# facebookresearch/goliath

Measured on NVIDIA H100. Metric: rendered megapixels/sec (fwd+bwd) RGCA head 300k Gaussians, higher is better.
Workload: dtype f32

## Files before the change

### goliath_b200/_lib.py

```python
import ctypes
import os

import torch

_HERE = os.path.dirname(os.path.abspath(__file__))
LIB_PATH = os.path.join(_HERE, "libgoliath_b200.so")
_lib = None

_vp, _i, _f, _i64, _sz = ctypes.c_void_p, ctypes.c_int, ctypes.c_float, ctypes.c_int64, ctypes.c_size_t

SIGNATURES = {
    "gb_version": (_i, []),
    "gb_launch_count": (ctypes.c_ulonglong, []),
    "gb_launch_count_reset": (None, []),
    "gb_sg_evaluate_fwd": (_i, [_vp] * 7 + [_i] * 4 + [_vp]),
    "gb_sg_evaluate_bwd": (_i, [_vp] * 10 + [_i] * 4 + [_vp]),
    "gb_project_gaussians_fwd": (_i, [_i, _vp, _vp, _f, _vp, _vp, _f, _f, _f, _f, _i, _i, _i, _f] + [_vp] * 7 + [_vp]),
    "gb_project_gaussians_bwd": (_i, [_i, _vp, _vp, _f, _vp, _vp, _f, _f] + [_vp] * 13 + [_vp]),
    "gb_cumsum_workspace_bytes": (_sz, [_i]),
    "gb_cumsum_i32": (_i, [_i, _vp, _vp, _vp, _vp]),
    "gb_map_gaussian_to_intersects": (_i, [_i, _vp, _vp, _vp, _vp, _i, _i, _i, _vp, _vp, _vp]),
    "gb_sort_workspace_bytes": (_sz, [_i64]),
    "gb_sort_intersects": (_i, [_i64, _vp, _vp, _vp, _vp, _i, _vp, _vp]),
    "gb_get_tile_bin_edges": (_i, [_i64, _vp, _vp, _vp]),
# ... 11 lines not shown
    "gb_get_rank_sort_mode": (_i, []),
    "gb_set_rank_sort_mode": (None, [_i]),
    "gb_bin_tiles_supported": (_i, [_i]),
    "gb_bin_tiles_workspace_bytes": (_sz, [_i, _i, _i64]),
    "gb_bin_tiles_pack": (_i, [_i] + [_vp] * 7 + [_i, _i, _i, _i64] + [_vp, _vp, _i] + [_vp] * 5 + [_vp]),
    "gb_bin_tiles_pack_ev": (_i, [_i] + [_vp] * 7 + [_i, _i, _i, _i64] + [_vp, _vp, _i] + [_vp] * 5 + [_vp, _vp]),
    "gb_tile_schedule_ints": (_i, [_i]),
    "gb_tile_schedule": (_i, [_i, _vp, _vp, _vp]),
    "gb_rasterize_sched_fwd": (_i, [_i, _i, _i] + [_vp] * 7 + [_vp]),
    "gb_rasterize_sched_bwd": (_i, [_i, _i, _i] + [_vp] * 13 + [_vp]),
    "gb_records_widen": (_i, [_i64, _vp, _vp, _vp, _vp]),
    "gb_records_set_colors4": (_i, [_i64, _vp, _vp, _vp, _i, _i64, _vp, _vp]),
    "gb_rasterize_multi_fwd": (_i, [_i, _i, _vp, _vp, _i, _vp, _vp, _vp, _vp]),
    "gb_rasterize_multi_bwd": (_i, [_i, _i, _vp, _vp, _vp, _i] + [_vp] * 9 + [_vp]),
    "gb_colors12_unpack": (_i, [_i64, _i, _vp, _vp, _vp]),
    "gb_records_set_colors": (_i, [_i64] + [_vp] * 5 + [_vp]),
    "gb_splat_grad_unpack": (_i, [_i] + [_vp] * 8 + [_vp]),
    "gb_get_blend_mode": (_i, []),
    "gb_set_blend_mode": (None, [_i]),
    "gb_rasterize_packed_fwd": (_i, [_i, _i, _i] + [_vp] * 7 + [_vp]),
    "gb_rasterize_packed_bwd": (_i, [_i, _i, _i] + [_vp] * 13 + [_vp]),
    "gb_rasterize_ranked_fwd": (_i, [_i, _i, _i] + [_vp] * 8 + [_vp]),
    "gb_rasterize_ranked_bwd": (_i, [_i, _i, _i] + [_vp] * 14 + [_vp]),
    "gb_bin_tiles_ranked": (_i, [_i] + [_vp] * 7 + [_i, _i, _i, _i64] + [_vp, _vp, _i] + [_vp] * 6 + [_vp, _vp]),
    "gb_compute_raydirs_fwd": (_i, [_i, _i, _i] + [_vp] * 5 + [_f] + [_vp] * 3 + [_vp]),
    "gb_compute_raydirs_bwd": (_i, []),
    "gb_mvp_aabb_workspace_bytes": (_sz, [_i, _i]),
    "gb_mvp_compute_aabb": (_i, [_i, _i] + [_vp] * 8 + [_vp]),
    "gb_get_raymarch_mode": (_i, []),
    "gb_set_raymarch_mode": (None, [_i]),
    "gb_mvp_raymarch_fwd": (_i, [_i] * 4 + [_vp, _vp, _f] + [_vp] * 5 + [_i] * 3 + [_vp] + [_i] * 3 + [_vp] * 4
                            + [_i, _f, _f, _i, _i, _vp]),
    "gb_deconv_tc_weight_bytes": (_sz, [_i, _i]),
    "gb_nchw_to_nhwc_split": (_i, [_i] * 5 + [_vp] * 3 + [_vp]),
    "gb_deconv4x4s2_tc_fwd": (_i, [_i] * 6 + [_vp] * 6 + [_f, _i, _vp, _vp, _i, _vp, _vp]),
    "gb_deconv4x4s2_wnub_fwd": (_i, [_i] * 5 + [_vp] * 4 + [_f, _i, _vp, _vp]),
    "gb_deconv4x4s2_wnub_bwd": (_i, [_i] * 5 + [_vp] * 5 + [_f, _i] + [_vp] * 4 + [_vp]),
    "gb_conv4x4s2_wnub_fwd": (_i, [_i] * 5 + [_vp] * 4 + [_f, _i, _vp, _vp]),
    "gb_conv4x4s2_wnub_bwd": (_i, [_i] * 5 + [_vp] * 5 + [_f, _i] + [_vp] * 4 + [_vp]),
    "gb_conv2d_wnub_fwd": (_i, [_i] * 6 + [_vp] * 4 + [_i, _f, _i, _vp, _vp]),
    "gb_conv2d_wnub_bwd": (_i, [_i] * 6 + [_vp] * 5 + [_f, _i, _i] + [_vp] * 4 + [_vp]),
    "gb_mvp_slab_to_prims_fwd": (_i, [_i] * 6 + [_vp] * 3 + [_f, _f, _i, _vp, _vp]),
    "gb_mvp_slab_to_prims_bwd": (_i, [_i] * 6 + [_vp] * 3 + [_f, _f, _i] + [_vp] * 3 + [_vp]),
    "gb_mvp_prim_transform_fwd": (_i, [_i, _i] + [_vp] * 3 + [_f, _i] + [_vp] * 3 + [_vp]),
    "gb_mvp_prim_transform_bwd": (_i, [_i, _i] + [_vp] * 3 + [_f, _i] + [_vp] * 4 + [_vp]),
    "gb_mvp_prim_frames_fwd": (_i, [_i] * 4 + [_vp] * 10 + [_vp]),
# ... 76 lines not shown
```

### goliath_b200/csrc/splat_blend_mom.cu

```cuda
#include <cstdlib>
#include <cstring>

#include "common.cuh"
#include "splat_blend_common.cuh"

namespace {

using namespace gbblend;

constexpr int kPixelWarps = 8;
constexpr int kStageRecs = 128;
constexpr int kFwdStages = 4;
constexpr int kFwdThreads = (kPixelWarps + 1) * 32;
constexpr int kBwdStages = 3;
constexpr int kBwdThreads = kPixelWarps * 32;
constexpr int kChunk = 16;
constexpr int kEntryCap = 48;
constexpr int kMStride = 33;
constexpr float kCullMargin = 2e-3f;

__device__ __forceinline__ float rcp_approx(float x) {
  float r;
  asm("rcp.approx.ftz.f32 %0, %1;" : "=f"(r) : "f"(x));
  return r;
// ... 21 lines not shown
  if (q0.z > 1e30f) return true;
  const float4 q1 = *q1p;
  const float dxlo = q0.x - fx1, dxhi = q0.x - fx0, dylo = q0.y - fy1, dyhi = q0.y - fy0;
  const float ex0 = fminf(fmaxf(0.f, dxlo), dxhi), ey0 = fminf(fmaxf(0.f, dylo), dyhi);
  const float dy1 = fminf(fmaxf(-q1.y * ex0 * rcp_approx(q1.z), dylo), dyhi);
  const float dx2 = fminf(fmaxf(-q1.y * ey0 * rcp_approx(q1.x), dxlo), dxhi);
  const float f1 = 0.5f * (q1.x * ex0 * ex0 + q1.z * dy1 * dy1) + q1.y * ex0 * dy1;
  const float f2 = 0.5f * (q1.x * dx2 * dx2 + q1.z * ey0 * ey0) + q1.y * dx2 * ey0;
  const float s = __logf(255.f * q1.w);
  return fminf(f1, f2) <= s + kCullMargin + 1e-4f * fabsf(s);
}

struct Tile {
  int tile_id, tx, ty;
};
__device__ __forceinline__ Tile make_tile(int tile_id, int tbx) {
  Tile t;
  t.tile_id = tile_id;
  t.ty = tile_id / tbx;
  t.tx = tile_id - t.ty * tbx;
  return t;
}

template <int C, bool LIST, bool RANKED>
__global__ void __launch_bounds__(kFwdThreads) blend_fwd_ilp_kernel(
    int img_w, int img_h, int tbx, const int* order, int sched, const int2* __restrict__ tile_bins,
    const float4* __restrict__ rec , const int* __restrict__ ranks ,
    const float* __restrict__ background, float* __restrict__ final_Ts, int* __restrict__ final_idx,
    float* __restrict__ out_img) {
  __shared__ __align__(128) float4 s_rec[kFwdStages][kStageRecs * 3];
  __shared__ __align__(8) unsigned long long s_full[kFwdStages];
  __shared__ __align__(8) unsigned long long s_empty[kFwdStages];
  __shared__ int s_ndone;
  __shared__ int s_tile;
  __shared__ __align__(16) int s_hits[LIST ? kPixelWarps : 1][LIST ? kStageRecs + 4 : 4];

  const int tr = threadIdx.x, lane = tr & 31, warp = tr >> 5;
  if (tr == 0) {
    s_tile = draw_tile(order, sched, tbx * ((img_h + 15) >> 4));
#pragma unroll
    for (int s = 0; s < kFwdStages; ++s) {
      mbar_init(&s_full[s], RANKED ? 32 : 1);
      mbar_init(&s_empty[s], kPixelWarps);
    }
    s_ndone = 0;
    fence_mbar_init();
  }
  __syncthreads();
  if (s_tile < 0) return;
  const Tile tl = make_tile(s_tile, tbx);
  const int2 range = tile_bins[tl.tile_id];
  const int num_batches = (range.y - range.x + kStageRecs - 1) / kStageRecs;
// ... 49 lines not shown
        if (*ndone >= kPixelWarps) break;
      }
      const int start = range.x + b * kStageRecs;
      const unsigned bytes = (unsigned)min(kStageRecs, range.y - start) * kRecBytes;
      mbar_expect_tx(&s_full[s], bytes);
      bulk_g2s(&s_rec[s][0], rec + (size_t)start * 3, bytes, &s_full[s]);
      issued = b + 1;
    }
    for (int b = max(0, issued - kFwdStages); b < issued; ++b)
      mbar_wait(&s_full[b % kFwdStages], (unsigned)((b / kFwdStages) & 1));
    return;
  }

  const int wx0 = tl.tx * 16 + ((warp & 1) << 3), wy0 = tl.ty * 16 + ((warp >> 1) << 2);
  const int pxi = wx0 + (lane & 7), pyi = wy0 + (lane >> 3);
  const bool inside = (pxi < img_w) && (pyi < img_h);
  const float px = (float)pxi + 0.5f, py = (float)pyi + 0.5f;
  const float fx0 = (float)wx0 + 0.5f, fx1 = (float)wx0 + 7.5f, fy0 = (float)wy0 + 0.5f, fy1 = (float)wy0 + 3.5f;

  bool done = !inside;
  float T = 1.f;
  int cur_idx = 0;
  float acc[4] = {0.f, 0.f, 0.f, 0.f};

  bool counted = false;
  for (int b = 0; b < num_batches; ++b) {
    const bool all_done = __all_sync(0xffffffffu, done);
    if (all_done && !counted) {
      counted = true;
      if (lane == 0) atomicAdd(&s_ndone, 1);
    }
    const int s = b % kFwdStages;
    const unsigned par = (unsigned)((b / kFwdStages) & 1);
    int st = 0;
    if (lane == 0) {
      volatile int* ndone = &s_ndone;
      for (;;) {
        if (mbar_try(&s_full[s], par)) { st = 1; break; }
        if (all_done && *ndone >= kPixelWarps) { st = 2; break; }
      }
    }
    st = __shfl_sync(0xffffffffu, st, 0);
    if (st == 2) break;
    if (all_done) {
      if (lane == 0) mbar_arrive(&s_empty[s]);
      continue;
    }
    mbar_wait(&s_full[s], par);
    const float4* sr = s_rec[s];
    const int batch_start = range.x + b * kStageRecs;
    const int batch_size = min(kStageRecs, range.y - batch_start);
    if (LIST) {
      int* hl = s_hits[LIST ? warp : 0];
      const unsigned lt = (1u << lane) - 1u;
      int cnt = 0;
#pragma unroll 4
      for (int c0 = 0; c0 < batch_size; c0 += 32) {
        const int ti = c0 + lane;
        bool hit = false;
        if (ti < batch_size) hit = footprint_hit(sr[ti * 3], &sr[ti * 3 + 1], fx0, fx1, fy0, fy1);
        const unsigned mask = __ballot_sync(0xffffffffu, hit);
        if (hit) hl[cnt + __popc(mask & lt)] = ti;
        cnt += __popc(mask);
      }
      __syncwarp();
      for (int i0 = 0; i0 < cnt; i0 += 16) {
        const int i1 = min(i0 + 16, cnt);
        for (int i = i0; i < i1; i += 4) {
          const int4 e = *reinterpret_cast<const int4*>(hl + i);
          bool live[4];
          int t[4];
          live[0] = true; live[1] = i + 1 < cnt; live[2] = i + 2 < cnt; live[3] = i + 3 < cnt;
          t[0] = e.x; t[1] = live[1] ? e.y : e.x; t[2] = live[2] ? e.z : e.x; t[3] = live[3] ? e.w : e.x;
          float alpha[4], sig[4];
          float4 col[4];
#pragma unroll
          for (int u = 0; u < 4; ++u) {
            const float4 q0 = sr[t[u] * 3], q1 = sr[t[u] * 3 + 1];
            col[u] = sr[t[u] * 3 + 2];
            const float dx = q0.x - px, dy = q0.y - py;
            sig[u] = 0.5f * (q1.x * dx * dx + q1.z * dy * dy) + q1.y * dx * dy;
            alpha[u] = fminf(kAlphaMaxFwd, q1.w * exp_neg(sig[u]));
          }
#pragma unroll
          for (int u = 0; u < 4; ++u) {
            const bool ok = live[u] && !done && !(sig[u] < 0.f) && !(alpha[u] < kAlphaMin);
            const float next_T = T * (1.f - alpha[u]);
            const bool stop = ok && (next_T <= kTEps);
            const bool take = ok && !stop;
            done = done || stop;
            if (take) {
              const float vis = alpha[u] * T;
              acc[0] += col[u].x * vis;
              acc[1] += col[u].y * vis;
              acc[2] += col[u].z * vis;
              if (C == 4) acc[3] += col[u].w * vis;
              T = next_T;
              cur_idx = batch_start + t[u];
            }
          }
        }
        if (__all_sync(0xffffffffu, done)) break;
      }
    } else {
    for (int c0 = 0; c0 < batch_size; c0 += 32) {
        const int ti = c0 + lane;
        bool hit = false;
        if (ti < batch_size) hit = footprint_hit(sr[ti * 3], &sr[ti * 3 + 1], fx0, fx1, fy0, fy1);
        unsigned mask = __ballot_sync(0xffffffffu, hit);
        while (mask) {
          int t[4];
          bool live[4];
  #pragma unroll
          for (int u = 0; u < 4; ++u) {
            live[u] = mask != 0;
            t[u] = live[u] ? c0 + __ffs(mask) - 1 : t[0];
            mask &= mask - 1;
          }
          float alpha[4], sig[4];
          float4 col[4];
  #pragma unroll
          for (int u = 0; u < 4; ++u) {
            const float4 q0 = sr[t[u] * 3], q1 = sr[t[u] * 3 + 1];
            col[u] = sr[t[u] * 3 + 2];
            const float dx = q0.x - px, dy = q0.y - py;
            sig[u] = 0.5f * (q1.x * dx * dx + q1.z * dy * dy) + q1.y * dx * dy;
// ... 3 lines not shown
          for (int u = 0; u < 4; ++u) {
            const bool ok = live[u] && !done && !(sig[u] < 0.f) && !(alpha[u] < kAlphaMin);
            const float next_T = T * (1.f - alpha[u]);
            const bool stop = ok && (next_T <= kTEps);
            const bool take = ok && !stop;
            done = done || stop;
            if (take) {
              const float vis = alpha[u] * T;
              acc[0] += col[u].x * vis;
              acc[1] += col[u].y * vis;
              acc[2] += col[u].z * vis;
              if (C == 4) acc[3] += col[u].w * vis;
              T = next_T;
              cur_idx = batch_start + t[u];
            }
          }
        }
        if (__all_sync(0xffffffffu, done)) break;
      }
  }
    __syncwarp();
    if (lane == 0) mbar_arrive(&s_empty[s]);
  }
  if (inside) {
    const size_t pix = (size_t)pyi * img_w + pxi;
    final_Ts[pix] = T;
    final_idx[pix] = cur_idx;
    if (C == 4) {
      reinterpret_cast<float4*>(out_img)[pix] =
          make_float4(acc[0] + T * background[0], acc[1] + T * background[1], acc[2] + T * background[2],
                      acc[3] + T * background[3]);
    } else {
      out_img[pix * 3 + 0] = acc[0] + T * background[0];
      out_img[pix * 3 + 1] = acc[1] + T * background[1];
      out_img[pix * 3 + 2] = acc[2] + T * background[2];
    }
  }
}

constexpr int kSmRec = kBwdStages * kStageRecs * kRecBytes;
constexpr int kSmEntries = kPixelWarps * kEntryCap * 48;
constexpr int kSmM = kPixelWarps * kChunk * kMStride * 8;
constexpr int kSmVo = kPixelWarps * 32 * 16;
constexpr int kBwdSmem = kSmRec + kSmEntries + kSmM + kSmVo;

template <int C, bool RANKED>
// ... 272 lines not shown
    __syncwarp();
    int refill = 0;
    if (lane == 0) {
      __threadfence_block();
      const int ticket = atomicAdd(&s_ticket[s], 1);
      if (ticket == kPixelWarps - 1) {
        __threadfence_block();
        s_ticket[s] = 0;
        if (k + kBwdStages < num_batches) {
          if (RANKED) refill = 1;
          else issue(k + kBwdStages);
        }
      }
    }
    if (RANKED) {
      refill = __shfl_sync(0xffffffffu, refill, 0);
      if (refill) issue_ranked(k + kBwdStages);
    }
  }
  if (cnt > 0) chunk(0, pad4(cnt));
  if (RANKED) cp_async_wait_all();
}

constexpr int kMK = 4;
constexpr int kMC = 3 * kMK;
constexpr int kMRQ = 5;
constexpr int kMRecBytes = kMRQ * 16;

__global__ void __launch_bounds__(kFwdThreads) blend_fwd_multi_kernel(
    int img_w, int img_h, int tbx, const int* order, int sched, const int2* __restrict__ tile_bins,
    const float4* __restrict__ rec, const float* __restrict__ background, float* __restrict__ out_planes ) {
  __shared__ __align__(128) float4 s_rec[kFwdStages][kStageRecs * kMRQ];
  __shared__ __align__(8) unsigned long long s_full[kFwdStages];
  __shared__ __align__(8) unsigned long long s_empty[kFwdStages];
  __shared__ int s_ndone;
  __shared__ __align__(16) int s_hits[kPixelWarps][kStageRecs + 4];
  __shared__ int s_tile;

  const int tr = threadIdx.x, lane = tr & 31, warp = tr >> 5;
  if (tr == 0) {
    s_tile = draw_tile(order, sched, tbx * ((img_h + 15) >> 4));
#pragma unroll
    for (int s = 0; s < kFwdStages; ++s) {
      mbar_init(&s_full[s], 1);
      mbar_init(&s_empty[s], kPixelWarps);
    }
// ... 423 lines not shown
    if (k < nk) {
      float* dst = v_colors + ((size_t)k * G + g) * 3;
      dst[0] = v[3 * k]; dst[1] = v[3 * k + 1]; dst[2] = v[3 * k + 2];
    }
  const float4 z = make_float4(0.f, 0.f, 0.f, 0.f);
  v12[3 * g] = z; v12[3 * g + 1] = z; v12[3 * g + 2] = z;
}

bool g_multi_attr_set[64] = {};

bool g_attr_set[64] = {};

}

namespace gbblend {

static bool fwd_list_variant() {
  const char* e = getenv("GOLIATH_B200_BLEND_FWD");
  return !(e && !strcmp(e, "rounds"));
}

static int launch_fwd_any(int img_h, int img_w, int channels, const int32_t* tile_bins, const int32_t* tile_order, int sched,
                          const float* records, const int32_t* ranks, const float* background, float* out_img,
                          float* final_Ts, int32_t* final_idx, cudaStream_t s) {
  const int tbx = gb::cdiv(img_w, 16), tby = gb::cdiv(img_h, 16);
  if (sched && !tile_order) return (int)cudaErrorInvalidValue;
  static const bool list = fwd_list_variant();
#define GB_FWD_MOM(CC, LL, RR)                                                                                          \
  blend_fwd_ilp_kernel<CC, LL, RR><<<tbx * tby, kFwdThreads, 0, s>>>(img_w, img_h, tbx, tile_order, sched,              \
                                                                     (const int2*)tile_bins, (const float4*)records,    \
                                                                     ranks, background, final_Ts, final_idx, out_img)
  if (ranks) {
    if (channels == 3) GB_FWD_MOM(3, true, true); else GB_FWD_MOM(4, true, true);
  } else if (channels == 3) {
    if (list) GB_FWD_MOM(3, true, false); else GB_FWD_MOM(3, false, false);
  } else {
    if (list) GB_FWD_MOM(4, true, false); else GB_FWD_MOM(4, false, false);
  }
#undef GB_FWD_MOM
  gb::count_launches(1);
  GB_CHECK_LAUNCH();
  return 0;
}

static int launch_bwd_any(int img_h, int img_w, int channels, const int32_t* gids_sorted, const int32_t* ranks,
                          const int32_t* tile_bins, const int32_t* tile_order, int sched, const float* records,
                          const float* background, const float* final_Ts, const int32_t* final_idx, const float* v_output,
                          const float* v_output_alpha, float* v_xy, float* v_conic, float* v_colors, float* v_opacity,
                          cudaStream_t s) {
  const int tbx = gb::cdiv(img_w, 16), tby = gb::cdiv(img_h, 16);
  if (sched && !tile_order) return (int)cudaErrorInvalidValue;
  int dev = 0;
  GB_CUDA(cudaGetDevice(&dev));
  if (dev < 0 || dev >= 64 || !g_attr_set[dev]) {
    GB_CUDA(cudaFuncSetAttribute(blend_bwd_mom_kernel<3, false>, cudaFuncAttributeMaxDynamicSharedMemorySize, kBwdSmem));
    GB_CUDA(cudaFuncSetAttribute(blend_bwd_mom_kernel<4, false>, cudaFuncAttributeMaxDynamicSharedMemorySize, kBwdSmem));
    GB_CUDA(cudaFuncSetAttribute(blend_bwd_mom_kernel<3, true>, cudaFuncAttributeMaxDynamicSharedMemorySize, kBwdSmem));
    GB_CUDA(cudaFuncSetAttribute(blend_bwd_mom_kernel<4, true>, cudaFuncAttributeMaxDynamicSharedMemorySize, kBwdSmem));
    if (dev >= 0 && dev < 64) g_attr_set[dev] = true;
  }
#define GB_BWD_MOM(CC, RR)                                                                                              \
  blend_bwd_mom_kernel<CC, RR><<<tbx * tby, kBwdThreads, kBwdSmem, s>>>(                                                \
      img_w, img_h, tbx, tile_order, sched, gids_sorted, ranks, (const int2*)tile_bins, (const float4*)records, background, \
      final_Ts, final_idx, v_output, v_output_alpha, v_xy, v_conic, v_colors, v_opacity)
  if (ranks) {
    if (channels == 3) GB_BWD_MOM(3, true); else GB_BWD_MOM(4, true);
  } else {
    if (channels == 3) GB_BWD_MOM(3, false); else GB_BWD_MOM(4, false);
  }
#undef GB_BWD_MOM
  gb::count_launches(1);
  GB_CHECK_LAUNCH();
  return 0;
}

int launch_fwd_mom(int img_h, int img_w, int channels, const int32_t* tile_bins, const int32_t* tile_order, int sched,
                   const float* records, const float* background, float* out_img, float* final_Ts, int32_t* final_idx,
                   cudaStream_t s) {
  return launch_fwd_any(img_h, img_w, channels, tile_bins, tile_order, sched, records, nullptr, background, out_img, final_Ts,
                        final_idx, s);
}

int launch_bwd_mom(int img_h, int img_w, int channels, const int32_t* gids_sorted, const int32_t* tile_bins,
                   const int32_t* tile_order, int sched, const float* records, const float* background, const float* final_Ts,
                   const int32_t* final_idx, const float* v_output, const float* v_output_alpha, float* v_xy,
                   float* v_conic, float* v_colors, float* v_opacity, cudaStream_t s) {
  return launch_bwd_any(img_h, img_w, channels, gids_sorted, nullptr, tile_bins, tile_order, sched, records, background,
                        final_Ts, final_idx, v_output, v_output_alpha, v_xy, v_conic, v_colors, v_opacity, s);
}

}

GB_API int gb_rasterize_ranked_fwd(int img_h, int img_w, int channels, const int32_t* tile_bins, const int32_t* tile_order,
                                   const int32_t* ranks_sorted, const float* rec_by_rank, const float* background,
                                   float* out_img, float* final_Ts, int32_t* final_idx, void* stream) {
  if (img_h <= 0 || img_w <= 0) return 0;
  if ((channels != 3 && channels != 4) || !ranks_sorted) return (int)cudaErrorInvalidValue;
  return gbblend::launch_fwd_any(img_h, img_w, channels, tile_bins, tile_order, 0, rec_by_rank, ranks_sorted, background,
                                 out_img, final_Ts, final_idx, (cudaStream_t)stream);
}
GB_API int gb_rasterize_ranked_bwd(int img_h, int img_w, int channels, const int32_t* rank_to_gid,
                                   const int32_t* ranks_sorted, const int32_t* tile_bins, const int32_t* tile_order,
                                   const float* rec_by_rank, const float* background, const float* final_Ts,
                                   const int32_t* final_idx, const float* v_output, const float* v_output_alpha,
                                   float* v_xy, float* v_conic, float* v_colors, float* v_opacity, void* stream) {
  if (img_h <= 0 || img_w <= 0) return 0;
  if ((channels != 3 && channels != 4) || !ranks_sorted) return (int)cudaErrorInvalidValue;
  return gbblend::launch_bwd_any(img_h, img_w, channels, rank_to_gid, ranks_sorted, tile_bins, tile_order, 0, rec_by_rank,
                                 background, final_Ts, final_idx, v_output, v_output_alpha, v_xy, v_conic, v_colors,
                                 v_opacity, (cudaStream_t)stream);
}

GB_API int gb_records_widen(int64_t cap, const int32_t* n_dev, const float* records, float* records_wide, void* stream) {
  if (cap <= 0) return 0;
  records_widen_kernel<<<(unsigned)gb::cdiv64(cap, 256), 256, 0, (cudaStream_t)stream>>>(cap, n_dev, (const float4*)records,
                                                                                         (float4*)records_wide);
  gb::count_launches(1);
  GB_CHECK_LAUNCH();
  return 0;
}
GB_API int gb_records_set_colors4(int64_t cap, const int32_t* n_dev, const int32_t* gids_sorted, const float* colors, int nk,
                                  int64_t G, float* records_wide, void* stream) {
  if (cap <= 0) return 0;
  if (nk < 1 || nk > 4) return (int)cudaErrorInvalidValue;
  records_set_colors4_kernel<<<(unsigned)gb::cdiv64(cap, 256), 256, 0, (cudaStream_t)stream>>>(cap, n_dev, gids_sorted, colors, nk,
                                                                                               G, (float4*)records_wide);
  gb::count_launches(1);
  GB_CHECK_LAUNCH();
  return 0;
}
GB_API int gb_rasterize_multi_fwd(int img_h, int img_w, const int32_t* tile_bins, const int32_t* tile_order, int sched,
                                  const float* records_wide, const float* background, float* out_planes, void* stream) {
  if (img_h <= 0 || img_w <= 0) return 0;
// ... 37 lines not shown
```

### goliath_b200/gsplat/fused.py

```python
import os
from typing import NamedTuple

import torch
from torch.autograd import Function

from .. import _lib
from .project import _project_bwd, _project_fwd
from .utils import _tile_bounds, _workspace, bin_and_sort_gaussians, compute_cumulative_intersects, key_bits

_OVERFLOW = {}

BINNING = os.environ.get("GOLIATH_B200_BINNING", "buckets")
SPLIT = os.environ.get("GOLIATH_B200_RENDER_SPLIT", "1") != "0"
RANKED = os.environ.get("GOLIATH_B200_RECORDS", "ranked") == "ranked"


def _overflow_flag(dev):
    f = _OVERFLOW.get(dev.index)
    if f is None:
        f = torch.zeros(1, dtype=torch.int32, device=dev)
        _OVERFLOW[dev.index] = f
    return f


# ... 205 lines not shown
        out4 = torch.empty(H, W, 4, **f32)
        final_Ts = torch.empty(H, W, **f32)
        final_idx = torch.empty(H, W, **i32)
        bg4 = torch.cat([background, background[:1]])
        tb = _tile_bounds(H, W, 16)
        cap = int(capacity)
        plan = _blend_plan(tb[0] * tb[1])
        ev = None
        if colors_event is not None:
            ev = colors_event.cuda_event
            colors.record_stream(torch.cuda.current_stream(dev))
        if plan.ranked:
            gids = torch.empty(G, **i32)
            ranks = torch.empty(cap, **i32)
            records = torch.empty(G, 12, **f32)
            outs = (ranks, records, gids)
        else:
            gids = torch.empty(cap, **i32)
            ranks = gids
            records = torch.empty(cap, 12, **f32)
            outs = (gids, records)
        bins, order = _bin_tiles(xys, depths, radii, conics, colors, opacity, comp, H, W, cap, plan, outs,
                                 ranked=plan.ranked, colors_ready=ev)
        with torch.cuda.device(dev):
            st = _lib.stream_ptr(dev)
            if plan.ranked:
                _lib.check(L.gb_rasterize_ranked_fwd(H, W, 4, _lib.ptr(bins), _lib.ptr(order), _lib.ptr(ranks),
                                                     _lib.ptr(records), _lib.ptr(bg4), _lib.ptr(out4), _lib.ptr(final_Ts),
                                                     _lib.ptr(final_idx), st), "rasterize_ranked_forward")
            else:
                _lib.check(plan.fwd(H, W, 4, _lib.ptr(bins), _lib.ptr(order), _lib.ptr(records), _lib.ptr(bg4),
                                    _lib.ptr(out4), _lib.ptr(final_Ts), _lib.ptr(final_idx), st),
                           "rasterize_packed_forward")
        ctx.save_for_backward(opacity, comp, bg4, gids, bins, order, records, final_Ts, final_idx, ranks)
        ctx.meta = (H, W, plan)
        ctx.set_materialize_grads(False)
        return out4, 1 - final_Ts

    @staticmethod
    def backward(ctx, v_out4, v_alpha):
        opacity, comp, bg4, gids, bins, order, records, final_Ts, final_idx, ranks = ctx.saved_tensors
        H, W, plan = ctx.meta

        def blend(st, *grads):
            if plan.ranked:
                _lib.check(_lib.lib().gb_rasterize_ranked_bwd(
                    H, W, 4, _lib.ptr(gids), _lib.ptr(ranks), _lib.ptr(bins), _lib.ptr(order), _lib.ptr(records),
                    _lib.ptr(bg4), _lib.ptr(final_Ts), _lib.ptr(final_idx), *map(_lib.ptr, grads), st),
                    "rasterize_ranked_backward")
            else:
                _lib.check(plan.bwd(H, W, 4, _lib.ptr(gids), _lib.ptr(bins), _lib.ptr(order), _lib.ptr(records),
                                    _lib.ptr(bg4), _lib.ptr(final_Ts), _lib.ptr(final_idx), *map(_lib.ptr, grads), st),
                           "rasterize_packed_backward")

        v_xy, v_conic, v_colors, v_opacity, v_comp, v_depth = _blend_grads(H, W, v_out4, v_alpha, opacity, comp, blend)
        return (v_xy, v_depth, v_conic, v_comp, None, v_opacity, v_colors) + (None,) * 5


def render_fused_split(means3d, scales, glob_scale, quats, viewmat, fx, fy, cx, cy, img_height, img_width, opacity, colors,
                       background, clip_thresh, capacity, colors_event=None):
    xys, depths, conics, comp, radii = _ProjectGeom.apply(means3d, scales, quats, viewmat, glob_scale, fx, fy, cx, cy,
                                                          img_height, img_width, clip_thresh)
    out4, alpha = _BinBlend.apply(xys, depths, conics, comp, radii, opacity, colors, background, img_height, img_width,
                                  capacity, colors_event)
    return out4, alpha, radii


def render_fused(means3d, scales, glob_scale, quats, viewmat, fx, fy, cx, cy, img_height, img_width, opacity, colors,
                 background, clip_thresh=0.01, capacity=None, colors_event=None):
    if (capacity is not None and SPLIT and BINNING == "buckets" and means3d.size(0) > 0
            and _lib.lib().gb_bin_tiles_supported(means3d.size(0))):
        return render_fused_split(means3d, scales, glob_scale, quats, viewmat, fx, fy, cx, cy, img_height, img_width,
# ... 6 lines not shown
```

### include/goliath_b200.h

```cpp
#ifndef GOLIATH_B200_H_
#define GOLIATH_B200_H_

#include <stddef.h>
#include <stdint.h>

#ifdef __cplusplus
extern "C" {
#endif

int gb_version(void);
unsigned long long gb_launch_count(void);
void gb_launch_count_reset(void);


int gb_sg_evaluate_fwd(const float* lobe_dirs, const float* lobe_sigmas, const float* light_values,
                       const float* light_pts, const float* prim_pts, const int32_t* n_lights, float* integral,
                       int N, int D, int L, int w_type, void* stream);

int gb_sg_evaluate_bwd(const float* lobe_dirs, const float* lobe_sigmas, const float* light_values,
                       const float* light_pts, const float* prim_pts, const int32_t* n_lights,
                       const float* grad_integral, float* grad_dirs, float* grad_sigmas, float* grad_light_values,
                       int N, int D, int L, int w_type, void* stream);


// ... 82 lines not shown
                      const float* colors3, const float* opacity, const float* compensation, int img_h, int img_w,
                      int block_width, int64_t cap, int32_t* tile_bins, int32_t* tile_order, int tile_sched,
                      int32_t* gids_sorted, float* records, int32_t* n_out, int32_t* overflow, void* workspace,
                      void* stream);
int gb_bin_tiles_pack_ev(int G, const float* xys, const float* depths, const int32_t* radii, const float* conics,
                         const float* colors3, const float* opacity, const float* compensation, int img_h, int img_w,
                         int block_width, int64_t cap, int32_t* tile_bins, int32_t* tile_order, int tile_sched,
                         int32_t* gids_sorted, float* records, int32_t* n_out, int32_t* overflow, void* workspace,
                         void* colors_ready, void* stream);

int gb_bin_tiles_ranked(int G, const float* xys, const float* depths, const int32_t* radii, const float* conics,
                        const float* colors3, const float* opacity, const float* compensation, int img_h, int img_w,
                        int block_width, int64_t cap, int32_t* tile_bins, int32_t* tile_order, int tile_sched,
                        int32_t* ranks_sorted, float* rec_by_rank, int32_t* rank_to_gid, int32_t* n_out, int32_t* overflow,
                        void* workspace, void* colors_ready, void* stream);
int gb_rasterize_ranked_fwd(int img_h, int img_w, int channels, const int32_t* tile_bins, const int32_t* tile_order,
                            const int32_t* ranks_sorted, const float* rec_by_rank, const float* background,
                            float* out_img, float* final_Ts, int32_t* final_idx, void* stream);
int gb_rasterize_ranked_bwd(int img_h, int img_w, int channels, const int32_t* rank_to_gid, const int32_t* ranks_sorted,
                            const int32_t* tile_bins, const int32_t* tile_order, const float* rec_by_rank,
                            const float* background, const float* final_Ts, const int32_t* final_idx,
                            const float* v_output, const float* v_output_alpha, float* v_xy, float* v_conic,
                            float* v_colors, float* v_opacity, void* stream);

int gb_tile_order(int num_tiles, const int32_t* tile_bins, int32_t* order, void* stream);

int gb_get_blend_mode(void);
void gb_set_blend_mode(int mode);

int gb_tile_schedule_ints(int num_tiles);
int gb_tile_schedule(int num_tiles, const int32_t* tile_bins, int32_t* sched, void* stream);
int gb_rasterize_sched_fwd(int img_h, int img_w, int channels, const int32_t* tile_bins, int32_t* sched,
                           const float* records, const float* background, float* out_img, float* final_Ts,
                           int32_t* final_idx, void* stream);
int gb_rasterize_sched_bwd(int img_h, int img_w, int channels, const int32_t* gids_sorted, const int32_t* tile_bins,
                           int32_t* sched, const float* records, const float* background, const float* final_Ts,
                           const int32_t* final_idx, const float* v_output, const float* v_output_alpha, float* v_xy,
                           float* v_conic, float* v_colors, float* v_opacity, void* stream);

int gb_rasterize_packed_fwd(int img_h, int img_w, int channels, const int32_t* tile_bins, const int32_t* tile_order,
                            const float* records, const float* background, float* out_img, float* final_Ts,
                            int32_t* final_idx, void* stream);

int gb_rasterize_packed_bwd(int img_h, int img_w, int channels, const int32_t* gids_sorted,
                            const int32_t* tile_bins, const int32_t* tile_order, const float* records,
                            const float* background, const float* final_Ts, const int32_t* final_idx,
// ... 179 lines not shown
```

Measured before the change: 1518.

## Record per-warp hit lists in forward and replay them in backward blend

The forward blend kernel now writes each warp's list of Gaussians that actually passed the coverage test, plus a per-warp count, into new buffers. A new backward kernel walks only those recorded hits in reverse instead of re-scanning every Gaussian in the tile. It also takes work items dynamically from a queue ordered by list length, so long lists start first. This adds forward-pass writes and an 8x-capacity hit buffer in memory, and needs an extra single-block ordering kernel launch.

New measurement: 1596, median of 6. 1.05x the previous value.

```diff
diff --git a/goliath_b200/_lib.py b/goliath_b200/_lib.py
--- a/goliath_b200/_lib.py
+++ b/goliath_b200/_lib.py
@@ -57,6 +57,8 @@
     "gb_rasterize_packed_bwd": (_i, [_i, _i, _i] + [_vp] * 13 + [_vp]),
     "gb_rasterize_ranked_fwd": (_i, [_i, _i, _i] + [_vp] * 8 + [_vp]),
     "gb_rasterize_ranked_bwd": (_i, [_i, _i, _i] + [_vp] * 14 + [_vp]),
+    "gb_rasterize_ranked_fwd_lists": (_i, [_i, _i, _i] + [_vp] * 10 + [_vp]),
+    "gb_rasterize_ranked_bwd_lists": (_i, [_i, _i, _i] + [_vp] * 14 + [_vp]),
     "gb_bin_tiles_ranked": (_i, [_i] + [_vp] * 7 + [_i, _i, _i, _i64] + [_vp, _vp, _i] + [_vp] * 6 + [_vp, _vp]),
     "gb_compute_raydirs_fwd": (_i, [_i, _i, _i] + [_vp] * 5 + [_f] + [_vp] * 3 + [_vp]),
     "gb_compute_raydirs_bwd": (_i, []),
diff --git a/goliath_b200/csrc/splat_blend_mom.cu b/goliath_b200/csrc/splat_blend_mom.cu
--- a/goliath_b200/csrc/splat_blend_mom.cu
+++ b/goliath_b200/csrc/splat_blend_mom.cu
@@ -67,12 +67,13 @@
   return t;
 }
 
-template <int C, bool LIST, bool RANKED>
+template <int C, bool LIST, bool RANKED, bool HITS = false>
 __global__ void __launch_bounds__(kFwdThreads) blend_fwd_ilp_kernel(
     int img_w, int img_h, int tbx, const int* order, int sched, const int2* __restrict__ tile_bins,
     const float4* __restrict__ rec , const int* __restrict__ ranks ,
     const float* __restrict__ background, float* __restrict__ final_Ts, int* __restrict__ final_idx,
-    float* __restrict__ out_img) {
+    float* __restrict__ out_img, int* __restrict__ hit_list = nullptr, int* __restrict__ hit_count = nullptr) {
+  static_assert(!HITS || LIST, "hit lists are the LIST variant's per-stage lists");
   __shared__ __align__(128) float4 s_rec[kFwdStages][kStageRecs * 3];
   __shared__ __align__(8) unsigned long long s_full[kFwdStages];
   __shared__ __align__(8) unsigned long long s_empty[kFwdStages];
@@ -168,6 +169,8 @@
   float T = 1.f;
   int cur_idx = 0;
   float acc[4] = {0.f, 0.f, 0.f, 0.f};
+  int* const seg = HITS ? hit_list + 8 * (size_t)range.x + (size_t)warp * (range.y - range.x) : nullptr;
+  int written = 0, last_pos = -1;
 
   bool counted = false;
   for (int b = 0; b < num_batches; ++b) {
@@ -210,6 +213,10 @@
         cnt += __popc(mask);
       }
       __syncwarp();
+      if (HITS) {
+        for (int i = lane; i < cnt; i += 32) seg[written + i] = batch_start + hl[i];
+        if (b == 0 && range.x == 0 && cnt > 0 && hl[0] == 0 && inside) last_pos = 0;
+      }
       for (int i0 = 0; i0 < cnt; i0 += 16) {
         const int i1 = min(i0 + 16, cnt);
         for (int i = i0; i < i1; i += 4) {
@@ -243,11 +250,13 @@
               if (C == 4) acc[3] += col[u].w * vis;
               T = next_T;
               cur_idx = batch_start + t[u];
+              if (HITS) last_pos = written + i + u;
             }
           }
         }
         if (__all_sync(0xffffffffu, done)) break;
       }
+      written += cnt;
     } else {
     for (int c0 = 0; c0 < batch_size; c0 += 32) {
         const int ti = c0 + lane;
@@ -297,6 +306,12 @@
     __syncwarp();
     if (lane == 0) mbar_arrive(&s_empty[s]);
   }
+  if (HITS) {
+#pragma unroll
+    for (int o = 16; o > 0; o >>= 1) last_pos = max(last_pos, __shfl_xor_sync(0xffffffffu, last_pos, o));
+    if (lane == 0) hit_count[8 * tl.tile_id + warp] = last_pos + 1;
+    if (blockIdx.x == 0 && tr == 0) hit_count[8 * tbx * ((img_h + 15) >> 4)] = 0;
+  }
   if (inside) {
     const size_t pix = (size_t)pyi * img_w + pxi;
     final_Ts[pix] = T;
@@ -615,6 +630,237 @@
   if (RANKED) cp_async_wait_all();
 }
 
+constexpr int kListWarps = 4;
+constexpr int kListThreads = kListWarps * 32;
+constexpr int kOrderBuckets = 64;
+
+__device__ __forceinline__ void cp_async_commit() { asm volatile("cp.async.commit_group;" ::: "memory"); }
+
+__global__ void __launch_bounds__(1024) order_items_kernel(int n_items, int* __restrict__ hit_count) {
+  __shared__ int s_off[kOrderBuckets];
+  const int tr = threadIdx.x, lane = tr & 31;
+  auto bucket = [](int n) { return kOrderBuckets - 1 - min((n + kChunk - 1) / kChunk, kOrderBuckets - 1); };
+  if (tr < kOrderBuckets) s_off[tr] = 0;
+  __syncthreads();
+  for (int i = tr; i < n_items; i += blockDim.x) {
+    const int n = hit_count[i];
+    if (n > 0) atomicAdd(&s_off[bucket(n)], 1);
+  }
+  __syncthreads();
+  if (tr < 32) {
+    const int a = s_off[2 * lane], b = s_off[2 * lane + 1];
+    int incl = a + b;
+#pragma unroll
+    for (int o = 1; o < 32; o <<= 1) {
+      const int t = __shfl_up_sync(0xffffffffu, incl, o);
+      if (lane >= o) incl += t;
+    }
+    const int excl = incl - a - b;
+    s_off[2 * lane] = excl;
+    s_off[2 * lane + 1] = excl + a;
+    if (lane == 31) hit_count[n_items + 1] = incl;
+  }
+  __syncthreads();
+  int* items = hit_count + n_items + 2;
+  for (int i = tr; i < n_items; i += blockDim.x) {
+    const int n = hit_count[i];
+    if (n > 0) items[atomicAdd(&s_off[bucket(n)], 1)] = i;
+  }
+}
+
+template <int C>
+__global__ void __launch_bounds__(kListThreads, 6) blend_bwd_lists_kernel(
+    int img_w, int img_h, int tbx, int n_items, const int2* __restrict__ tile_bins, const int* __restrict__ hit_list,
+    const int* __restrict__ hit_count, int* draw ,
+    const int* __restrict__ ranks, const float4* __restrict__ rec, const float* __restrict__ background,
+    const float* __restrict__ final_Ts, const int* __restrict__ final_idx, const float* __restrict__ v_output,
+    const float* __restrict__ v_output_alpha, float* __restrict__ v_xy, float* __restrict__ v_conic,
+    float* __restrict__ v_colors, float* __restrict__ v_opacity) {
+  __shared__ __align__(16) float4 s_e[kListWarps][2][kChunk * 3];
+  __shared__ __align__(8) int2 s_ig[kListWarps][2][kChunk];
+  __shared__ float2 s_m[kListWarps][kChunk * kMStride];
+  __shared__ float4 s_vo[kListWarps][32];
+
+  const int lane = threadIdx.x & 31, wib = threadIdx.x >> 5;
+  float2* M = s_m[wib];
+  float4* VO = s_vo[wib];
+  const int n_work = hit_count[n_items + 1];
+  const int* items = hit_count + n_items + 2;
+  const int n_draws = n_work + (int)gridDim.x * kListWarps;
+  for (;;) {
+    int k = 0;
+    if (lane == 0) {
+      k = atomicAdd(draw, 1);
+      if (k == n_draws - 1) *draw = 0;
+    }
+    k = __shfl_sync(0xffffffffu, k, 0);
+    if (k >= n_work) break;
+    const int item = items[k], tile = item >> 3, warp = item & 7;
+    const int n = hit_count[item];
+    const int2 range = tile_bins[tile];
+    const int* list = hit_list + 8 * (size_t)range.x + (size_t)warp * (range.y - range.x);
+    const Tile tl = make_tile(tile, tbx);
+    const int wx0 = tl.tx * 16 + ((warp & 1) << 3), wy0 = tl.ty * 16 + ((warp >> 1) << 2);
+    const int pxi = wx0 + (lane & 7), pyi = wy0 + (lane >> 3);
+    const bool inside = (pxi < img_w) && (pyi < img_h);
+    const float px = (float)pxi + 0.5f, py = (float)pyi + 0.5f;
+    const float fx0 = (float)wx0 + 0.5f, fy0 = (float)wy0 + 0.5f;
+    const size_t pix = inside ? ((size_t)pyi * img_w + pxi) : 0;
+
+    const int nchunks = (n + kChunk - 1) / kChunk;
+    int g_idx = 0, g_id = 0;
+    auto load_next = [&](int j) {
+      const int top = n - kChunk * j;
+      if (lane < min(kChunk, top)) {
+        g_idx = list[top - 1 - lane];
+        g_id = ranks[g_idx];
+      }
+    };
+    auto gather = [&](int j) {
+      const int cnt = min(kChunk, n - kChunk * j);
+      float4* E = s_e[wib][j & 1];
+      if (lane < cnt) {
+        const float4* src = rec + 3 * (size_t)g_id;
+        cp_async16(&E[lane * 3 + 0], src);
+        cp_async16(&E[lane * 3 + 1], src + 1);
+        cp_async16(&E[lane * 3 + 2], src + 2);
+        s_ig[wib][j & 1][lane] = make_int2(g_idx, g_id);
+      } else if (lane < ((cnt + 3) & ~3)) {
+        E[lane * 3 + 0] = make_float4(0.f, 0.f, 0.f, 0.f);
+        E[lane * 3 + 1] = make_float4(1.f, 0.f, 1.f, 0.f);
+        E[lane * 3 + 2] = make_float4(0.f, 0.f, 0.f, 0.f);
+        s_ig[wib][j & 1][lane] = make_int2(0x7fffffff, 0);
+      }
+      cp_async_commit();
+    };
+    load_next(0);
+    gather(0);
+
+    const float T_final = inside ? final_Ts[pix] : 1.f;
+    float T = T_final;
+    float bufv = 0.f;
+    const int bin_final = inside ? final_idx[pix] : -1;
+    float vo[4] = {0.f, 0.f, 0.f, 0.f};
+    float voa = 0.f;
+    if (inside) {
+#pragma unroll
+      for (int c = 0; c < C; ++c) vo[c] = v_output[pix * C + c];
+      voa = v_output_alpha ? v_output_alpha[pix] : 0.f;
+    }
+    VO[lane] = make_float4(vo[0], vo[1], vo[2], vo[3]);
+    float bgdot = 0.f;
+#pragma unroll
+    for (int c = 0; c < C; ++c) bgdot += background[c] * vo[c];
+    const float tfc = T_final * (voa - bgdot);
+    if (nchunks > 1) load_next(1);
+
+    for (int j = 0; j < nchunks; ++j) {
+      const int cnt = min(kChunk, n - kChunk * j);
+      const int nn = j + 1 < nchunks ? kChunk : ((cnt + 3) & ~3);
+      const float4* E = s_e[wib][j & 1];
+      const int2* IG = s_ig[wib][j & 1];
+      cp_async_wait_all();
+      __syncwarp();
+#pragma unroll 1
+      for (int h0 = 0; h0 < nn; h0 += 4) {
+        float al[4], ov[4], ra[4];
+        float4 col[4];
+#pragma unroll
+        for (int u = 0; u < 4; ++u) {
+          const int h = h0 + u;
+          const float4 q0 = E[h * 3], q1 = E[h * 3 + 1];
+          col[u] = E[h * 3 + 2];
+          const float dx = q0.x - px, dy = q0.y - py;
+          const float sigma = 0.5f * (q1.x * dx * dx + q1.z * dy * dy) + q1.y * dx * dy;
+          const float vis = exp_neg(sigma);
+          const float alpha = fminf(kAlphaMaxBwd, q1.w * vis);
+          const bool valid = (IG[h].x <= bin_final) && !(sigma < 0.f) && !(alpha < kAlphaMin);
+          al[u] = valid ? alpha : 0.f;
+          ov[u] = valid ? q1.w * vis : 0.f;
+          ra[u] = rcp_approx(1.f - al[u]);
+        }
+#pragma unroll
+        for (int u = 0; u < 4; ++u) {
+          const float cc[4] = {col[u].x, col[u].y, col[u].z, col[u].w};
+          float cv = 0.f;
+#pragma unroll
+          for (int c = 0; c < C; ++c) cv += cc[c] * vo[c];
+          const float v_alpha = ((cv * T - bufv) + tfc) * ra[u];
+          T *= ra[u];
+          const float fac = al[u] * T;
+          bufv += cv * fac;
+          M[(h0 + u) * kMStride + lane] = make_float2(fac, -ov[u] * v_alpha);
+        }
+      }
+      if (j + 1 < nchunks) {
+        gather(j + 1);
+        if (j + 2 < nchunks) load_next(j + 2);
+      }
+      __syncwarp();
+      {
+        const int hh = lane & 15, half = lane >> 4;
+        const int he = min(hh, nn - 1);
+        const float4 q0 = E[he * 3], q1 = E[he * 3 + 1];
+        const int e_id = IG[he].y;
+        const float2* Mrow = M + hh * kMStride + half * 16;
+        const float4* V = VO + half * 16;
+        float g[4] = {0.f, 0.f, 0.f, 0.f};
+        float r00 = 0.f, r01 = 0.f, r10 = 0.f, r11 = 0.f, sii = 0.f;
+        float facmax = 0.f;
+#pragma unroll
+        for (int q = 0; q < 16; ++q) {
+          const float2 m = Mrow[q];
+          const float4 v = V[q];
+          const float fi = (float)(q & 7);
+          facmax = fmaxf(facmax, m.x);
+          g[0] += m.x * v.x;
+          g[1] += m.x * v.y;
+          g[2] += m.x * v.z;
+          if (C == 4) g[3] += m.x * v.w;
+          if (q < 8) {
+            r00 += m.y;
+            r10 += m.y * fi;
+          } else {
+            r01 += m.y;
+            r11 += m.y * fi;
+          }
+          sii += m.y * (fi * fi);
+        }
+        const float u_ = q0.x - fx0, v_ = q0.y - (fy0 + (float)(2 * half));
+        const float S0 = r00 + r01, Sj = r01, Si = r10 + r11, Sij = r11;
+        const float sx = u_ * S0 - Si, sy = v_ * S0 - Sj;
+        const float sxx = u_ * (u_ * S0 - 2.f * Si) + sii;
+        const float sxy = u_ * (v_ * S0 - Sj) - v_ * Si + Sij;
+        const float syy = v_ * (v_ * S0 - 2.f * Sj) + Sj;
+        float o[10];
+        o[0] = g[0]; o[1] = g[1]; o[2] = g[2]; o[3] = g[3];
+        o[4] = 0.5f * sxx; o[5] = sxy; o[6] = 0.5f * syy;
+        o[7] = q1.x * sx + q1.y * sy;
+        o[8] = q1.y * sx + q1.z * sy;
+        o[9] = S0;
+#pragma unroll
+        for (int i = 0; i < 10; ++i) o[i] += __shfl_xor_sync(0xffffffffu, o[i], 16);
+        facmax = fmaxf(facmax, __shfl_xor_sync(0xffffffffu, facmax, 16));
+        if (half == 0 && hh < nn && facmax > 0.f) {
+          if (C == 4) {
+            gb::red_add_v4(v_colors + 4 * (size_t)e_id, o[0], o[1], o[2], o[3]);
+          } else {
+            gb::red_add(v_colors + 3 * (size_t)e_id + 0, o[0]);
+            gb::red_add(v_colors + 3 * (size_t)e_id + 1, o[1]);
+            gb::red_add(v_colors + 3 * (size_t)e_id + 2, o[2]);
+          }
+          gb::red_add(v_conic + 3 * (size_t)e_id + 0, o[4]);
+          gb::red_add(v_conic + 3 * (size_t)e_id + 1, o[5]);
+          gb::red_add(v_conic + 3 * (size_t)e_id + 2, o[6]);
+          gb::red_add_v2(v_xy + 2 * (size_t)e_id, o[7], o[8]);
+          gb::red_add(v_opacity + e_id, -o[9] * rcp_approx(q1.w));
+        }
+      }
+      __syncwarp();
+    }
+  }
+}
+
 constexpr int kMK = 4;
 constexpr int kMC = 3 * kMK;
 constexpr int kMRQ = 5;
@@ -1084,15 +1330,18 @@
 
 static int launch_fwd_any(int img_h, int img_w, int channels, const int32_t* tile_bins, const int32_t* tile_order, int sched,
                           const float* records, const int32_t* ranks, const float* background, float* out_img,
-                          float* final_Ts, int32_t* final_idx, cudaStream_t s) {
+                          float* final_Ts, int32_t* final_idx, cudaStream_t s, int32_t* hit_list = nullptr,
+                          int32_t* hit_count = nullptr) {
   const int tbx = gb::cdiv(img_w, 16), tby = gb::cdiv(img_h, 16);
   if (sched && !tile_order) return (int)cudaErrorInvalidValue;
   static const bool list = fwd_list_variant();
-#define GB_FWD_MOM(CC, LL, RR)                                                                                          \
-  blend_fwd_ilp_kernel<CC, LL, RR><<<tbx * tby, kFwdThreads, 0, s>>>(img_w, img_h, tbx, tile_order, sched,              \
-                                                                     (const int2*)tile_bins, (const float4*)records,    \
-                                                                     ranks, background, final_Ts, final_idx, out_img)
-  if (ranks) {
+#define GB_FWD_MOM(CC, LL, RR, ...)                                                                                     \
+  blend_fwd_ilp_kernel<CC, LL, RR, ##__VA_ARGS__><<<tbx * tby, kFwdThreads, 0, s>>>(                                   \
+      img_w, img_h, tbx, tile_order, sched, (const int2*)tile_bins, (const float4*)records, ranks, background, final_Ts, \
+      final_idx, out_img, hit_list, hit_count)
+  if (ranks && hit_list) {
+    if (channels == 3) GB_FWD_MOM(3, true, true, true); else GB_FWD_MOM(4, true, true, true);
+  } else if (ranks) {
     if (channels == 3) GB_FWD_MOM(3, true, true); else GB_FWD_MOM(4, true, true);
   } else if (channels == 3) {
     if (list) GB_FWD_MOM(3, true, false); else GB_FWD_MOM(3, false, false);
@@ -1136,6 +1385,41 @@
   return 0;
 }
 
+static int launch_bwd_lists(int img_h, int img_w, int channels, const int32_t* ranks, const int32_t* tile_bins,
+                            const int32_t* hit_list, int32_t* hit_count, const float* records,
+                            const float* background, const float* final_Ts, const int32_t* final_idx,
+                            const float* v_output, const float* v_output_alpha, float* v_xy, float* v_conic,
+                            float* v_colors, float* v_opacity, cudaStream_t s) {
+  const int tbx = gb::cdiv(img_w, 16), tby = gb::cdiv(img_h, 16);
+  const int n_items = 8 * tbx * tby;
+  int dev = 0;
+  GB_CUDA(cudaGetDevice(&dev));
+  static int resident[64][2] = {};
+  int uncached = 0;
+  int& per_sm = (dev >= 0 && dev < 64) ? resident[dev][channels == 4] : uncached;
+  if (per_sm == 0) {
+    int n = 0, sms = 0;
+    if (channels == 4)
+      GB_CUDA(cudaOccupancyMaxActiveBlocksPerMultiprocessor(&n, blend_bwd_lists_kernel<4>, kListThreads, 0));
+    else
+      GB_CUDA(cudaOccupancyMaxActiveBlocksPerMultiprocessor(&n, blend_bwd_lists_kernel<3>, kListThreads, 0));
+    GB_CUDA(cudaDeviceGetAttribute(&sms, cudaDevAttrMultiProcessorCount, dev));
+    per_sm = max(1, n) * sms;
+  }
+  const int grid = min(per_sm, gb::cdiv(n_items, kListWarps));
+  order_items_kernel<<<1, 1024, 0, s>>>(n_items, hit_count);
+#define GB_BWD_LISTS(CC)                                                                                                \
+  blend_bwd_lists_kernel<CC><<<grid, kListThreads, 0, s>>>(                                                             \
+      img_w, img_h, tbx, n_items, (const int2*)tile_bins, hit_list, hit_count, hit_count + n_items, ranks,              \
+      (const float4*)records, background, final_Ts, final_idx, v_output, v_output_alpha, v_xy, v_conic, v_colors,       \
+      v_opacity)
+  if (channels == 3) GB_BWD_LISTS(3); else GB_BWD_LISTS(4);
+#undef GB_BWD_LISTS
+  gb::count_launches(2);
+  GB_CHECK_LAUNCH();
+  return 0;
+}
+
 int launch_fwd_mom(int img_h, int img_w, int channels, const int32_t* tile_bins, const int32_t* tile_order, int sched,
                    const float* records, const float* background, float* out_img, float* final_Ts, int32_t* final_idx,
                    cudaStream_t s) {
@@ -1171,6 +1455,26 @@
   return gbblend::launch_bwd_any(img_h, img_w, channels, rank_to_gid, ranks_sorted, tile_bins, tile_order, 0, rec_by_rank,
                                  background, final_Ts, final_idx, v_output, v_output_alpha, v_xy, v_conic, v_colors,
                                  v_opacity, (cudaStream_t)stream);
+}
+GB_API int gb_rasterize_ranked_fwd_lists(int img_h, int img_w, int channels, const int32_t* tile_bins,
+                                         const int32_t* tile_order, const int32_t* ranks_sorted, const float* rec_by_rank,
+                                         const float* background, float* out_img, float* final_Ts, int32_t* final_idx,
+                                         int32_t* hit_list, int32_t* hit_count, void* stream) {
+  if (img_h <= 0 || img_w <= 0) return 0;
+  if ((channels != 3 && channels != 4) || !ranks_sorted || !hit_list || !hit_count) return (int)cudaErrorInvalidValue;
+  return gbblend::launch_fwd_any(img_h, img_w, channels, tile_bins, tile_order, 0, rec_by_rank, ranks_sorted, background,
+                                 out_img, final_Ts, final_idx, (cudaStream_t)stream, hit_list, hit_count);
+}
+GB_API int gb_rasterize_ranked_bwd_lists(int img_h, int img_w, int channels, const int32_t* ranks_sorted,
+                                         const int32_t* tile_bins, const int32_t* hit_list, int32_t* hit_count,
+                                         const float* rec_by_rank, const float* background, const float* final_Ts,
+                                         const int32_t* final_idx, const float* v_output, const float* v_output_alpha,
+                                         float* v_xy, float* v_conic, float* v_colors, float* v_opacity, void* stream) {
+  if (img_h <= 0 || img_w <= 0) return 0;
+  if ((channels != 3 && channels != 4) || !ranks_sorted || !hit_list || !hit_count) return (int)cudaErrorInvalidValue;
+  return gbblend::launch_bwd_lists(img_h, img_w, channels, ranks_sorted, tile_bins, hit_list, hit_count,
+                                   rec_by_rank, background, final_Ts, final_idx, v_output, v_output_alpha, v_xy, v_conic,
+                                   v_colors, v_opacity, (cudaStream_t)stream);
 }
 
 GB_API int gb_records_widen(int64_t cap, const int32_t* n_dev, const float* records, float* records_wide, void* stream) {
diff --git a/goliath_b200/gsplat/fused.py b/goliath_b200/gsplat/fused.py
--- a/goliath_b200/gsplat/fused.py
+++ b/goliath_b200/gsplat/fused.py
@@ -251,32 +251,38 @@
             outs = (gids, records)
         bins, order = _bin_tiles(xys, depths, radii, conics, colors, opacity, comp, H, W, cap, plan, outs,
                                  ranked=plan.ranked, colors_ready=ev)
+        hit_list = hit_count = None
         with torch.cuda.device(dev):
             st = _lib.stream_ptr(dev)
             if plan.ranked:
-                _lib.check(L.gb_rasterize_ranked_fwd(H, W, 4, _lib.ptr(bins), _lib.ptr(order), _lib.ptr(ranks),
-                                                     _lib.ptr(records), _lib.ptr(bg4), _lib.ptr(out4), _lib.ptr(final_Ts),
-                                                     _lib.ptr(final_idx), st), "rasterize_ranked_forward")
+                hit_list = torch.empty(8 * cap, **i32)
+                hit_count = torch.empty(16 * tb[0] * tb[1] + 2, **i32)
+                _lib.check(L.gb_rasterize_ranked_fwd_lists(H, W, 4, _lib.ptr(bins), _lib.ptr(order), _lib.ptr(ranks),
+                                                           _lib.ptr(records), _lib.ptr(bg4), _lib.ptr(out4),
+                                                           _lib.ptr(final_Ts), _lib.ptr(final_idx), _lib.ptr(hit_list),
+                                                           _lib.ptr(hit_count), st), "rasterize_ranked_forward")
             else:
                 _lib.check(plan.fwd(H, W, 4, _lib.ptr(bins), _lib.ptr(order), _lib.ptr(records), _lib.ptr(bg4),
                                     _lib.ptr(out4), _lib.ptr(final_Ts), _lib.ptr(final_idx), st),
                            "rasterize_packed_forward")
-        ctx.save_for_backward(opacity, comp, bg4, gids, bins, order, records, final_Ts, final_idx, ranks)
+        ctx.save_for_backward(opacity, comp, bg4, gids, bins, order, records, final_Ts, final_idx, ranks, hit_list,
+                              hit_count)
         ctx.meta = (H, W, plan)
         ctx.set_materialize_grads(False)
         return out4, 1 - final_Ts
 
     @staticmethod
     def backward(ctx, v_out4, v_alpha):
-        opacity, comp, bg4, gids, bins, order, records, final_Ts, final_idx, ranks = ctx.saved_tensors
+        (opacity, comp, bg4, gids, bins, order, records, final_Ts, final_idx, ranks, hit_list,
+         hit_count) = ctx.saved_tensors
         H, W, plan = ctx.meta
 
         def blend(st, *grads):
             if plan.ranked:
-                _lib.check(_lib.lib().gb_rasterize_ranked_bwd(
-                    H, W, 4, _lib.ptr(gids), _lib.ptr(ranks), _lib.ptr(bins), _lib.ptr(order), _lib.ptr(records),
-                    _lib.ptr(bg4), _lib.ptr(final_Ts), _lib.ptr(final_idx), *map(_lib.ptr, grads), st),
-                    "rasterize_ranked_backward")
+                _lib.check(_lib.lib().gb_rasterize_ranked_bwd_lists(
+                    H, W, 4, _lib.ptr(ranks), _lib.ptr(bins), _lib.ptr(hit_list),
+                    _lib.ptr(hit_count), _lib.ptr(records), _lib.ptr(bg4), _lib.ptr(final_Ts), _lib.ptr(final_idx),
+                    *map(_lib.ptr, grads), st), "rasterize_ranked_backward")
             else:
                 _lib.check(plan.bwd(H, W, 4, _lib.ptr(gids), _lib.ptr(bins), _lib.ptr(order), _lib.ptr(records),
                                     _lib.ptr(bg4), _lib.ptr(final_Ts), _lib.ptr(final_idx), *map(_lib.ptr, grads), st),
diff --git a/include/goliath_b200.h b/include/goliath_b200.h
--- a/include/goliath_b200.h
+++ b/include/goliath_b200.h
@@ -128,6 +128,16 @@
                             const float* background, const float* final_Ts, const int32_t* final_idx,
                             const float* v_output, const float* v_output_alpha, float* v_xy, float* v_conic,
                             float* v_colors, float* v_opacity, void* stream);
+int gb_rasterize_ranked_fwd_lists(int img_h, int img_w, int channels, const int32_t* tile_bins, const int32_t* tile_order,
+                                  const int32_t* ranks_sorted, const float* rec_by_rank, const float* background,
+                                  float* out_img, float* final_Ts, int32_t* final_idx, int32_t* hit_list,
+                                  int32_t* hit_count, void* stream);
+int gb_rasterize_ranked_bwd_lists(int img_h, int img_w, int channels, const int32_t* ranks_sorted,
+                                  const int32_t* tile_bins, const int32_t* hit_list,
+                                  int32_t* hit_count, const float* rec_by_rank, const float* background,
+                                  const float* final_Ts, const int32_t* final_idx, const float* v_output,
+                                  const float* v_output_alpha, float* v_xy, float* v_conic, float* v_colors,
+                                  float* v_opacity, void* stream);
 
 int gb_tile_order(int num_tiles, const int32_t* tile_bins, int32_t* order, void* stream);
 
```
